# G1OJS/PyFT8

Hardware: AMD Instinct MI355X
Metric: FT8 15-s frames decoded/sec (higher is better)
Workload: dtype f32

## Files before the change

pyft8_amd/csrc/ft8rx.hip:

```cpp
#include <hip/hip_runtime.h>
#include <math.h>
#include <stdarg.h>
#include <stdio.h>
#include <stdlib.h>
#include <string.h>
#include <algorithm>
#include <map>
#include <new>
#include <string>
#include <vector>
#include "../../include/ft8rx.h"
#include "ft8_dev.h"

#define WL_MULT(i) ((i) == WL_BP0 ? 5 : (i) == WL_OSDNAN ? 10 : 1)
#define NF0MAX (FT8RX_MAX_F0 > 1024 ? 2048 : 1024)

#include "kernels/common.hpp"
#include "kernels/spectrogram.hpp"
#include "kernels/sync_search.hpp"
#include "kernels/llr.hpp"
#include "kernels/ap_patterns.hpp"
#include "kernels/bp.hpp"
#include "kernels/cycle_spectrum.hpp"
#include "kernels/fine_sync.hpp"
// ... 585 lines not shown
static void launch_ap_calls(ft8rx_handle* h, int B, const float* llr0, ft8rx_record* rec, const int32_t* ncand, Att* attO, ft8rx_event* ev,
                            int32_t* evc, int32_t* cand_items, int32_t* osd_items, int32_t* ac, const ApCalls* apc, hipStream_t s) {
    const ft8rx_config& c = h->cfg;
    const int sh = cand_shift(c); const size_t S = (size_t)1 << sh;
    const int nflip = osd_nflip(c.osd_single, c.osd_triple);
    hipMemsetAsync(ac, 0, 2 * sizeof(int32_t), s);
    const WorkList cl = {cand_items, ac}, ol = {osd_items, ac + 1};
    k_ap_worklist<<<(B * S + 255) / 256, 256, 0, s>>>(rec, ncand, B, sh, cl);
    k_bp_ap<<<ladder_grid(h, B * c.max_cands * h->ap.np), 64, 0, s>>>(llr0, rec, ncand, attO, ev, evc, c, apc, cl, ol);
    (osd_wide(nflip) ? k_osd_ap_wide : k_osd_ap)<<<ladder_grid(h, B * c.max_cands * 3), 64, 0, s>>>(
        llr0, rec, ncand, attO, ev, evc, h->d_trials, h->n_trials, nflip, sh, apc, ol);
    k_select_ap<<<(B * S + 255) / 256, 256, 0, s>>>(rec, attO, apc, cl);
}

static void launch_reports(ft8rx_handle* h, int B, const cpx* spec, const ft8rx_record* rec, const int32_t* ncand, int32_t* items,
                           int32_t* count, ft8rx_report* rep, hipStream_t s) {
    const ft8rx_config& c = h->cfg;
    const int sh = cand_shift(c); const size_t S = (size_t)1 << sh;
    hipMemsetAsync(count, 0, sizeof(int32_t), s);
    const WorkList wl = {items, count};
    k_report_worklist<<<(B * S + 255) / 256, 256, 0, s>>>(rec, ncand, B, sh, wl, rep);
    k_report<<<ladder_grid(h, B * c.max_cands), FINE_NT, 0, s>>>(spec, rec, rep, h->T, sh, wl);
}

static void enqueue_chain(ft8rx_handle* h, const int16_t* d_audio, int f0, int B, hipStream_t s, bool prof, int slot, int chunk) {
    const ResultSlot& sl = h->slots[slot];
    const bool weak = h->weak;
    const ft8rx_config cw = weak ? weak_config(h) : h->cfg;
    const ft8rx_config& c = weak ? cw : h->cfg;
    const size_t F = (size_t)f0;
    const int sh = cand_shift(c); const size_t S = (size_t)1 << sh, FS = F * S;
    const int16_t* audio = d_audio + F * FT8RX_NSAMP;
    float* grid = h->d_grid + F * FT8RX_GRID_ROWS * FT8RX_GRID_COLS;
    float* bs = h->d_best_score + F * NF0MAX; int32_t* bh = h->d_best_h0 + F * NF0MAX;
    ft8rx_record* rec = sl.rec + FS; int32_t* ncand = sl.ncand + F;
    float* llr0 = h->d_llr0 + FS * 174; float* saved = h->d_saved + FS * 5 * 174;
    Att* att0 = h->d_att0 + FS * 5; Att* attG = h->d_attG + FS * 2; Att* attB = h->d_attB + FS * 5; Att* attO = h->d_attO + FS * 10;
    cpx* A = reinterpret_cast<cpx*>(grid); cpx* spec = A + (size_t)B * 96000;
    ft8rx_event* ev = sl.ev + F * FT8RX_EVENT_CAP; int32_t* evc = sl.evcount + F;
#define STAGE(name) do { if (prof) { hipEventRecord(h->pev[h->pnames.size()], s); h->pnames.push_back(name); } } while (0)
    int32_t* wc = h->d_wcount + WL_N * chunk;
    WorkList wl[WL_N];
    for (int i = 0; i < WL_N; i++) { wl[i].items = h->d_work[i] + FS * WL_MULT(i); wl[i].count = wc + i; }
    STAGE("spectrogram");
    ft8rx_ilp_spectrogram(B, s, audio, grid, h->T);
    STAGE("sync");
    launch_sync(grid, bs, bh, c, B, s, weak);
    STAGE("topk");
    k_topk<<<B, 1024, 0, s>>>(bs, bh, rec, ncand, c, evc, wc, h->use_mask ? h->d_colmask + F * NF0MAX : nullptr);
    STAGE("grid_llr");
    const unsigned mt = (unsigned)h->msg_types;
    launch_mt(k_grid_llr, k_grid_llr_ext, mt, XCD_GRID(B, c.max_cands), s, grid, rec, ncand, llr0, c, nullptr, nullptr, nullptr, att0, ev, evc, B);
    k_worklist_att<<<(B * S * 5 + 255) / 256, 256, 0, s>>>(rec, ncand, att0, B, sh, wl[WL_BP0]);
    STAGE("bp_grid");
    launch_mt(k_bp, k_bp_ext, mt, ladder_grid(h, B * c.max_cands * 5), s, 0, llr0, rec, ncand, nullptr, att0, nullptr, ev, evc, c, c.bp_nc0_a, c.bp_iters_a, wl[WL_BP0], 0, 5);
    STAGE("select0");
    k_select0<<<(B * S + 255) / 256, 256, 0, s>>>(rec, ncand, att0, B, sh, wl[WL_FINE]);
    STAGE("cycle_fft");
    k_cyc_a<<<dim3(40, B), 256, 0, s>>>(audio, A, h->T);
    k_cyc_bc<<<dim3(CYC_BC_GRID, B), 256, 0, s>>>(A, spec, h->T);
    STAGE("fine");
    launch_fine(h, c, weak, ladder_grid(h, B * c.max_cands), s, spec, rec, ncand, llr0, nullptr, nullptr, nullptr, nullptr, wl[WL_FINE],
                c.h0_lo < FT8RX_MIN_H0_FD || c.h0_hi > FT8RX_MAX_H0_FD + 1);
    k_worklist<<<(B * S + 255) / 256, 256, 0, s>>>(rec, ncand, B, sh, wl[WL_BP1]);
    STAGE("bp_fine");
    const auto bp_fine = [&](int n_variants, const WorkList& work, int v0) {
        launch_mt(k_bp, k_bp_ext, mt, B * c.max_cands * n_variants, s, 1, llr0, rec, ncand, attG, attB, saved, ev, evc, c, c.bp_nc0_b, c.bp_iters_b,
                  work, v0, n_variants);
    };
    if (h->ladder_mode == 0) {
        bp_fine(1, wl[WL_BP1], 0);
        k_select1<<<(B * S + 255) / 256, 256, 0, s>>>(0, rec, ncand, attG, attB, B, c, wl[WL_BP1B]);
        bp_fine(1, wl[WL_BP1B], 1);
        k_select1<<<(B * S + 255) / 256, 256, 0, s>>>(1, rec, ncand, attG, attB, B, c, wl[WL_BP1C]);
        bp_fine(3, wl[WL_BP1C], 2);
        STAGE("select1");
        k_select1<<<(B * S + 255) / 256, 256, 0, s>>>(2, rec, ncand, attG, attB, B, c, wl[WL_OSD]);
    } else {
        bp_fine(5, wl[WL_BP1], 0);
        STAGE("select1");
        k_select1<<<(B * S + 255) / 256, 256, 0, s>>>(3, rec, ncand, attG, attB, B, c, wl[WL_OSD]);
    }
    STAGE("osd");
    launch_osd(h, mt, ladder_grid(h, B * c.max_cands * 10), s, 0, llr0, saved, attB, rec, ncand, attO, ev, evc, h->d_trials, h->n_trials,
               osd_nflip(c.osd_single, c.osd_triple), c.osd_max_hd, sh, wl[WL_OSD], wl[WL_OSDNAN]);
    STAGE("select2");
    k_select2<<<(B * S + 255) / 256, 256, 0, s>>>(rec, ncand, attO, B, sh);
    if (h->ap.np) {
        STAGE("ap_calls");
        ApCalls* apc = h->d_apc + chunk;
        if (h->ap_chunk_version[chunk] != h->ap_version) {
            k_ap_stage<<<1, 64, 0, s>>>(apc, h->ap);
            h->ap_chunk_version[chunk] = h->ap_version;
        }
        launch_ap_calls(h, B, llr0, rec, ncand, attO, ev, evc, wl[WL_BP0].items, wl[WL_OSDNAN].items, h->d_apcount + 2 * chunk, apc, s);
    }
    if (sl.recall) {
        STAGE("recall");
        ft8rx_recall_entry* ent = sl.d_rc_ent + F * FT8RX_RECALL_MAX;
        int32_t* rcnt = sl.d_rc_cnt + F;
        k_recall_stage<<<B, FT8RX_RECALL_MAX, 0, s>>>(h->d_rc_src + F * FT8RX_RECALL_MAX, h->d_rc_srccnt + F, ent, rcnt, sl.d_rc_rec + F * FT8RX_RECALL_MAX);
        const int base = h->rc_off[F], n = h->rc_off[F + B] - base;
        if (n > 0) {
            k_recall_trip<<<B, FT8RX_RECALL_MAX, 0, s>>>(ent, rcnt, h->d_rc_off + F, h->d_rc_trip);
            const size_t b = (size_t)base;
            launch_fine(h, c, false, n, s, spec, nullptr, nullptr, h->d_rc_llr + b * 174, h->d_rc_trip + 3 * b, h->d_rc_tout + 5 * b,
                        h->d_rc_tsd + b, h->d_rc_sgrid + b * 632, WorkList{nullptr, nullptr}, h->rc_td);
            k_recall_score<<<n, 64, 0, s>>>(h->d_rc_sgrid, h->d_rc_tout, h->d_rc_trip, h->d_rc_off + F, base, ent, rec, ncand, sh,
                                            h->rc_max_hd, h->rc_min_gap, sl.d_rc_rec + F * FT8RX_RECALL_MAX);
        }
    }
    if (sl.reports) {
        STAGE("report");
        launch_reports(h, B, spec, rec, ncand, h->d_rp_items + FS, h->d_rp_count + chunk, sl.d_rp + FS, s);
    }
    if (prof) hipEventRecord(h->pev[h->pnames.size()], s);
#undef STAGE
}

static void enqueue_chunk(ft8rx_handle* h, const int16_t* d_audio, int f0, int n, hipStream_t s, int slot, int chunk) {
    const int sub = (h->sub_frames > 0 && h->sub_frames < n) ? h->sub_frames : n;
    for (int o = 0; o < n; o += sub) enqueue_chain(h, d_audio, f0 + o, (o + sub <= n) ? sub : n - o, s, false, slot, chunk);
}

using batchplan::BatchPlan;
using batchplan::Entry;

static int batch_begin(ft8rx_handle* h, Entry e, int B, int slot, bool chunked, int16_t** stage) {
    ResultSlot& sl = h->slots[slot];
    h->pnames.clear();
    if (e != batchplan::DEVICE && need_staging(h)) return -2;
    if (e == batchplan::HOST_PIPELINED && slot == 1 && need_staging(h, true)) return -2;
    if (h->inflight == 2) { h->slot_fetch ^= 1; h->inflight = 1; }
    if (h->rc_armed && B != h->rc_frames) { set_err(h, "recall entries were set for %d frames, the batch has %d", h->rc_frames, B); return -1; }
    sl.recall = h->rc_armed;
    h->rc_armed = false;
    sl.reports = h->reports;
    *stage = h->d_audio;
    if (e == batchplan::HOST_PIPELINED) {
        *stage = slot ? h->d_audio2 : h->d_audio;
        HIPCHK(h, hipStreamWaitEvent(h->h2d_s, sl.ev_comp, 0));
    }
    for (int i = 1; i < h->n_streams && chunked; i++) if (!h->sub[i - 1]) {
        if (!(h->sub[i - 1] = pool_sub(h->device, i - 1))) { set_err(h, "cannot create a chunk stream"); return -2; }
        HIPCHK(h, hipEventCreateWithFlags(&h->ev_join[i - 1], hipEventDisableTiming));
    }
    return 0;
}

static int batch_submit(ft8rx_handle* h, const BatchPlan& plan, Entry e, int slot, const int16_t* audio, int16_t* stage) {
    ResultSlot& sl = h->slots[slot];
    const bool host = e != batchplan::DEVICE;
    const int16_t* d_audio = host ? stage : audio; const int16_t* host_audio = host ? audio : nullptr;
    const int ns = h->n_streams, nc = plan.nc, B = plan.cb[nc];
    const bool free_run = plan.mode == batchplan::FREE_RUN, pipelined = e == batchplan::HOST_PIPELINED, sync_host = e == batchplan::HOST_SYNC;
    hipStream_t cs = pipelined ? h->h2d_s : h->copy_s;
    const size_t frame_bytes = sizeof(int16_t) * (size_t)FT8RX_NSAMP;
    auto chunk_stream = [&](int k) { const int i = k % ns; return i == 0 ? h->stream : h->sub[i - 1]; };
    if (free_run) {
        for (int i = 0; i < ns; i++) for (int k = 0; k < 2; k++)
            if (!h->ev_cdone[k][i]) HIPCHK(h, hipEventCreateWithFlags(&h->ev_cdone[k][i], hipEventDisableTiming));
        if (h->need_barrier || h->part_B != B || h->part_n != nc) {
            if (h->free_running) HIPCHK(h, hipStreamWaitEvent(h->stream, h->slots[h->last_slot].ev_comp, 0));
            HIPCHK(h, hipEventRecord(h->ev_fork, h->stream));
            for (int i = 1; i < ns; i++) HIPCHK(h, hipStreamWaitEvent(h->sub[i - 1], h->ev_fork, 0));
            h->need_barrier = false; h->part_B = B; h->part_n = nc;
        }
// ... 2078 lines not shown
```

pyft8_amd/csrc/kernels/osd.hpp:

```cpp
#ifndef FT8RX_OSD_HPP
#define FT8RX_OSD_HPP

#ifdef OSD_TIMING
__device__ unsigned long long g_osd_t[32768][10];
struct OsdClock { unsigned long long prev = __builtin_readcyclecounter(); };
#define OT(i) do { const unsigned long long ot_now = __builtin_readcyclecounter(); if (lane == 0) g_osd_t[blockIdx.x & 32767][i] += ot_now - ot.prev; ot.prev = __builtin_readcyclecounter(); } while (0)
#define OT_FLUSH do { if (lane == 0) g_osd_t[blockIdx.x & 32767][9] += 1ull; } while (0)
#else
struct OsdClock {};
#define OT(i) do { } while (0)
#define OT_FLUSH do { } while (0)
#endif
template <int M> FT8_DEV uint32_t osd_px(uint32_t v, int lane) {
    if (M == 1) return (uint32_t)__builtin_amdgcn_update_dpp(0, (int)v, 0xB1, 0xf, 0xf, false);
    if (M == 2) return (uint32_t)__builtin_amdgcn_update_dpp(0, (int)v, 0x4E, 0xf, 0xf, false);
    if (M == 3) return (uint32_t)__builtin_amdgcn_update_dpp(0, (int)v, 0x1B, 0xf, 0xf, false);
    if (M == 7) return (uint32_t)__builtin_amdgcn_update_dpp(0, (int)v, 0x141, 0xf, 0xf, false);
    if (M == 15) return (uint32_t)__builtin_amdgcn_update_dpp(0, (int)v, 0x140, 0xf, 0xf, false);
    if (M == 8) return (uint32_t)__builtin_amdgcn_update_dpp(0, (int)v, 0x128, 0xf, 0xf, false);
    if (M == 4 || M == 16 || M == 31) return (uint32_t)__builtin_amdgcn_ds_swizzle((int)v, 0x1f | (M << 10));
    return __shfl(v, lane ^ M);
}
#define OSD_LOWMASK(top) ((top) == 1 ? 0x5555555555555555ull : (top) == 2 ? 0x3333333333333333ull : (top) == 4 ? 0x0F0F0F0F0F0F0F0Full : \
                          (top) == 8 ? 0x00FF00FF00FF00FFull : (top) == 16 ? 0x0000FFFF0000FFFFull : 0x00000000FFFFFFFFull)
// ... 47 lines not shown
    const int val = a[last]; int next = last - 1;
    while (osd_nl(x, val, a[next])) { a[last] = a[next]; last = next; next--; }
    a[last] = val;
}
FT8_HD void osd_ss_insertion(const float* x, int* a, int first, int last) {
    for (int i = first + 1; i < last; i++) {
        if (osd_nl(x, a[i], a[first])) { const int val = a[i]; for (int j = i; j > first; j--) a[j] = a[j - 1]; a[first] = val; }
        else osd_ss_linear_insert(x, a, i);
    }
}
FT8_HD void osd_ss_adjust_heap(const float* x, int* a, int first, int hole, int len, int value) {
    const int top = hole; int child = hole;
    while (child < (len - 1) / 2) {
        child = 2 * (child + 1);
        if (osd_nl(x, a[first + child], a[first + child - 1])) child--;
        a[first + hole] = a[first + child]; hole = child;
    }
    if ((len & 1) == 0 && child == (len - 2) / 2) { child = 2 * (child + 1); a[first + hole] = a[first + child - 1]; hole = child - 1; }
    int parent = (hole - 1) / 2;
    while (hole > top && osd_nl(x, a[first + parent], value)) { a[first + hole] = a[first + parent]; hole = parent; parent = (hole - 1) / 2; }
    a[first + hole] = value;
}
FT8_HD void osd_std_sort_withnan(const float* x, int* a, int* stack ) {
    const int n = 174;
    for (int i = 0; i < n; i++) a[i] = i;
    int sp = 0;
    stack[0] = 0; stack[1] = n; stack[2] = 2 * 7; sp = 1;
    while (sp > 0) {
        sp--;
        int first = stack[3 * sp], last = stack[3 * sp + 1], depth = stack[3 * sp + 2];
        while (last - first > 16) {
            if (depth == 0) {
                const int len = last - first;
                for (int parent = (len - 2) / 2; parent >= 0; parent--) osd_ss_adjust_heap(x, a, first, parent, len, a[first + parent]);
                while (last - first > 1) { last--; const int v = a[last]; a[last] = a[first]; osd_ss_adjust_heap(x, a, first, 0, last - first, v); }
                break;
            }
            depth--;
            {
                const int p = first + 1, q = first + (last - first) / 2, r = last - 1;
                int pick;
                if (osd_nl(x, a[p], a[q])) pick = osd_nl(x, a[q], a[r]) ? q : (osd_nl(x, a[p], a[r]) ? r : p);
                else pick = osd_nl(x, a[p], a[r]) ? p : (osd_nl(x, a[q], a[r]) ? r : q);
                const int t = a[first]; a[first] = a[pick]; a[pick] = t;
            }
            int lo = first + 1, hi = last;
            for (;;) {
                while (osd_nl(x, a[lo], a[first])) lo++;
                hi--;
                while (osd_nl(x, a[first], a[hi])) hi--;
                if (!(lo < hi)) break;
                const int t = a[lo]; a[lo] = a[hi]; a[hi] = t;
                lo++;
            }
            stack[3 * sp] = lo; stack[3 * sp + 1] = last; stack[3 * sp + 2] = depth; sp++;
            last = lo;
        }
    }
    osd_ss_insertion(x, a, 0, 16);
    for (int i = 16; i < n; i++) osd_ss_linear_insert(x, a, i);
}

#undef FT8_HD
__device__ uint8_t d_NANPERM[192];

#define OSD_MAXFLIP 91
#define OSD_FLIPS_A 62
#define OSD_MAXTRIALS 16384
#define OSD_NONE 0xFFu

__device__ __constant__ uint32_t d_SYNM[14][3];
__device__ uint32_t d_G0T[192][3];

struct OsdArgs {
    const float* llr_in; const float* saved; const Att* attB; ft8rx_record* rec; const int32_t* ncand; Att* attO;
    ft8rx_event* ev; int32_t* evcount; const uint32_t* trials; int ntr, nflip, max_hd, sh; WorkList nanlist; unsigned mt; const ApCalls* apc;
};

struct OsdLds {
    float llr[176];
    uint64_t work[256];
    uint64_t ftab[192];
    uint32_t hmw[3];
    uint16_t fsyn[OSD_MAXFLIP + 2];
    FT8_DEV int* ordl() { return reinterpret_cast<int*>(work); }
    FT8_DEV int* posrow() { return reinterpret_cast<int*>(work); }
    FT8_DEV uint32_t* ftabB() { return reinterpret_cast<uint32_t*>(work); }
    FT8_DEV int* frow() { return reinterpret_cast<int*>(work) + 192; }
};
static_assert(176 + 3 * 20 <= 512 && 192 + OSD_MAXFLIP <= 512 && sizeof(OsdLds) <= 4496, "the overlays fit the 512 words of work[]; 4.5 KB per block");

struct OsdInput { bool go; int slot; size_t vec; const float* hsrc; };
template <bool AP7>
FT8_DEV OsdInput osd_load(OsdLds& L, int lane, int mode, int bid, const OsdArgs& a) {
    OsdInput in = {true, 0, (size_t)bid, L.llr};
    if constexpr (AP7) {
        in.slot = bid & 15; const size_t c = (size_t)(bid >> 4);
        in.hsrc = a.llr_in + c * 174;
        const float v0 = in.hsrc[lane], v1 = in.hsrc[64 + lane], v2 = in.hsrc[128 + (lane < 46 ? lane : 0)];
        L.llr[lane] = ap7_value(a.apc, in.slot, lane, v0); L.llr[64 + lane] = ap7_value(a.apc, in.slot, 64 + lane, v1);
        if (lane < 46) L.llr[128 + lane] = ap7_value(a.apc, in.slot, 128 + lane, v2);
        in.vec = c * 10 + (in.slot - 5);
    } else if (mode == 0) {
        const int slot = in.slot = bid % 10; const int c = bid / 10;
        in.go = false;
        if ((c & ((1 << a.sh) - 1)) >= a.ncand[c >> a.sh]) return in;
        if (a.rec[c].status != FT8RX_ST_ACTIVE) return in;
        if (slot >= 5 && !a.attB[(size_t)c * 5 + (slot - 5)].has_out) { if (lane == 0) { Att u; memset(&u, 0, sizeof(u)); u.n_its = -1; a.attO[(size_t)c * 10 + slot] = u; } return in; }
        in.go = true;
        const float* src = slot < 5 ? a.llr_in + (size_t)c * 174 : a.saved + ((size_t)c * 5 + (slot - 5)) * 174;
        const int apx = slot < 5 ? slot : 0;
        const float v0 = src[lane], v1 = src[64 + lane], v2 = src[128 + (lane < 46 ? lane : 0)];
        L.llr[lane] = ap_value(apx, lane, v0); L.llr[64 + lane] = ap_value(apx, 64 + lane, v1);
        if (lane < 46) L.llr[128 + lane] = ap_value(apx, 128 + lane, v2);
        in.vec = (size_t)c * 10 + slot;
    } else {
        for (int i = lane; i < 174; i += 64) L.llr[i] = a.llr_in[in.vec * 174 + i];
    }
    __syncthreads();
    return in;
}

template <bool NANV>
FT8_DEV bool osd_order(OsdLds& L, int lane, int bid, const WorkList& nanlist, uint32_t* ix, OsdClock& ot) {
    uint32_t hk[3];
#pragma unroll
    for (int q = 0; q < 3; q++) {
        const int i = lane + 64 * q;
        const uint32_t mag = __float_as_uint(L.llr[i < 174 ? i : 0]) & 0x7fffffffu;
        hk[q] = (i < 174) ? 0xFFFFFFFEu - mag : 0xFFFFFFFFu;
        ix[q] = (i < 174) ? (uint32_t)i : 0u;
    }
    const uint64_t nan0 = __ballot(hk[0] < 0x807FFFFEu), nan1 = __ballot(hk[1] < 0x807FFFFEu), nan2 = __ballot(lane < 46 && hk[2] < 0x807FFFFEu);
    const bool any_nan = (nan0 | nan1 | nan2) != 0, all_nan = (nan0 & nan1) == ~0ull && nan2 == (1ull << 46) - 1;
    OT(0);
    if (NANV) {
        if (!any_nan || all_nan) return false;
        int* ordl = L.ordl();
        if (lane == 0) osd_std_sort_withnan(L.llr, ordl, ordl + 176);
        __syncthreads();
        ix[0] = (uint32_t)ordl[lane]; ix[1] = (uint32_t)ordl[64 + lane]; ix[2] = (uint32_t)ordl[128 + (lane < 46 ? lane : 0)];
        __syncthreads();
    } else if (all_nan) {
        ix[0] = d_NANPERM[lane]; ix[1] = d_NANPERM[64 + lane]; ix[2] = d_NANPERM[128 + lane];
    } else if (any_nan) {
        if (lane == 0) work_push(nanlist, bid);
        return false;
    } else {
        osd_stage<1, 3>(hk, ix, lane); osd_stage<3, 3>(hk, ix, lane); osd_stage<1, 3>(hk, ix, lane);
        osd_stage<7, 3>(hk, ix, lane); osd_stage<2, 3>(hk, ix, lane); osd_stage<1, 3>(hk, ix, lane);
        osd_stage<15, 3>(hk, ix, lane); osd_stages_421<3>(hk, ix, lane);
        osd_stage<31, 3>(hk, ix, lane); osd_stage<8, 3>(hk, ix, lane); osd_stages_421<3>(hk, ix, lane);
        osd_stage<63, 3>(hk, ix, lane); osd_stage<16, 3>(hk, ix, lane); osd_stage<8, 3>(hk, ix, lane); osd_stages_421<3>(hk, ix, lane);
        osd_stage_regs<true>(hk[0], ix[0], hk[1], ix[1], lane);
        osd_stage<32, 2>(hk, ix, lane); osd_stage<16, 2>(hk, ix, lane); osd_stage<8, 2>(hk, ix, lane); osd_stages_421<2>(hk, ix, lane);
        osd_stage_regs<true>(hk[1], ix[1], hk[2], ix[2], lane);
        osd_stage_regs<false>(hk[0], ix[0], hk[1], ix[1], lane);
        osd_stage<32, 3>(hk, ix, lane); osd_stage<16, 3>(hk, ix, lane); osd_stage<8, 3>(hk, ix, lane); osd_stages_421<3>(hk, ix, lane);
    }
    return true;
}

struct OsdHard { uint64_t w0, w1, w2; };
FT8_DEV OsdHard osd_hard(const float* v, int lane) {
    return {__ballot(v[lane] > 0.0f), __ballot(v[64 + lane] > 0.0f), __ballot(lane < 46 && v[128 + (lane < 46 ? lane : 0)] > 0.0f)};
}

struct OsdBasis {
    uint32_t x00, x01, x02, x10, x11, x12, x20, x21, x22;
    uint64_t acc0, acc1, acc2;
    bool hs0, hs1, hs2;
};
FT8_DEV OsdBasis osd_eliminate(OsdLds& L, int lane, const uint32_t* ix, OsdClock& ot) {
    const int ord0 = (int)ix[0], ord1 = (int)ix[1], ord2 = (lane < 46) ? (int)ix[2] : 0;
    const bool has2 = lane < 46;
    uint32_t x00 = d_G0T[ord0][0], x01 = d_G0T[ord0][1], x02 = d_G0T[ord0][2];
    uint32_t x10 = d_G0T[ord1][0], x11 = d_G0T[ord1][1], x12 = d_G0T[ord1][2];
    uint32_t x20 = has2 ? d_G0T[ord2][0] : 0u, x21 = has2 ? d_G0T[ord2][1] : 0u, x22 = has2 ? d_G0T[ord2][2] : 0u;
    const bool hs0 = L.llr[ord0] > 0.0f, hs1 = L.llr[ord1] > 0.0f, hs2 = has2 && L.llr[ord2] > 0.0f;
    uint64_t acc0 = 0, acc1 = 0, acc2 = 0;
    int k = 0;
#define OSD_TRIV 96
    int* posrow = L.posrow();
    if (ord0 < 91) posrow[ord0] = lane;
    if (ord1 < 91) posrow[ord1] = 64 + lane;
    if (has2 && ord2 < 91) posrow[ord2] = 128 + lane;
    uint64_t triv0 = __ballot(ord0 < 91), triv1 = __ballot(ord1 < 91 && lane < OSD_TRIV - 64);
    int tc0 = __builtin_amdgcn_mbcnt_hi((uint32_t)(triv0 >> 32), __builtin_amdgcn_mbcnt_lo((uint32_t)triv0, 0));
    int tc1 = __popcll(triv0) + __builtin_amdgcn_mbcnt_hi((uint32_t)(triv1 >> 32), __builtin_amdgcn_mbcnt_lo((uint32_t)triv1, 0));
    int ntriv = __popcll(triv0) + __popcll(triv1);
    __syncthreads();
    const uint64_t u01 = __ballot(posrow[lane] < OSD_TRIV);
    const uint32_t u2 = (uint32_t)__ballot(lane < 27 && posrow[64 + (lane < 27 ? lane : 0)] < OSD_TRIV);
    uint64_t vis0 = ~triv0, vis1 = ~triv1, vis2 = (1ull << 46) - 1;
#define OSD_UPD(XW, X0, X1, X2) { const uint32_t mk = (uint32_t)__builtin_amdgcn_sbfe((int)(XW), bp, 1u); X0 ^= mk & m0; X1 ^= mk & m1; X2 ^= mk & m2; }
#define OSD_STEP(XA, XB, XC, ACC, VIS, TCV, BASE, UPD0, UPD1, UPD2)                                                                \
    while (VIS != 0) {                                                                                                             \
        const int il = __builtin_ctzll(VIS);                                                                                       \
        if (k + __builtin_amdgcn_readlane(TCV, il) >= 91) { vis0 = 0; vis1 = 0; vis2 = 0; continue; }       \
        const uint64_t bit = 1ull << il;                                                                                           \
        VIS &= ~bit; ACC |= bit; k++;                                                                                              \
        const uint32_t c0 = __builtin_amdgcn_readlane(XA, il), c1 = __builtin_amdgcn_readlane(XB, il), c2 = __builtin_amdgcn_readlane(XC, il); \
        uint32_t a0 = c0 & ~lockU0, a1 = c1 & ~lockU1, a2 = c2 & ~lockU2;                                                          \
        if (__builtin_expect(!(a0 | a1 | a2), 0)) {             \
            const int p = (BASE) + il;                                                                                             \
             \
            const int pa = posrow[lane], pb = posrow[64 + (lane < 27 ? lane : 0)];                                                 \
            const bool ta = pa > p && pa < OSD_TRIV && (((pa < 64 ? triv0 >> pa : triv1 >> (pa - 64)) & 1ull) != 0);               \
            const bool tb = lane < 27 && pb > p && pb < OSD_TRIV && (((pb < 64 ? triv0 >> pb : triv1 >> (pb - 64)) & 1ull) != 0);  \
            const uint64_t s01 = (((uint64_t)c1 << 32) | c0) & __ballot(ta);                                                       \
            a0 = (uint32_t)s01; a1 = (uint32_t)(s01 >> 32); a2 = c2 & (uint32_t)__ballot(tb);                                      \
            if (a0 | a1 | a2) {                                                                                                    \
                const int r = s01 ? __builtin_ctzll(s01) : 64 + __builtin_ctz(a2);                                                 \
                const int q = __builtin_amdgcn_readfirstlane(posrow[r]);    \
                if (q < 64) { triv0 &= ~(1ull << q); vis0 |= 1ull << q; tc0 -= (lane > q) ? 1 : 0; tc1 -= 1; }                    \
                else { triv1 &= ~(1ull << (q - 64)); vis1 |= 1ull << (q - 64); tc1 -= (lane > q - 64) ? 1 : 0; }                   \
                ntriv--;                                                                                                           \
            } else { ACC &= ~bit; k--; }                                                    \
        }                                                                                                                          \
        asm volatile("" : "+s"(a2));                            \
                        \
        if (a0) {                                                                                                                  \
            const uint32_t b = a0 & (0u - a0), bp = __builtin_ctz(a0), m0 = c0 & ~b, m1 = c1, m2 = c2;                             \
            UPD0                                                                                                                   \
            lockU0 |= b;                                                                                                           \
        } else if (a1) {                                                                                                           \
            const uint32_t b = a1 & (0u - a1), bp = __builtin_ctz(a1), m0 = c0, m1 = c1 & ~b, m2 = c2;                             \
            UPD1                                                                                                                   \
            lockU1 |= b;                                                                                                           \
        } else {                                                \
            const uint32_t b = a2 & (0u - a2), bp = __builtin_ctz(a2 | 0x80000000u), m0 = c0, m1 = c1, m2 = c2 & ~b;               \
            UPD2                                                                                                                   \
            lockU2 |= b;                                                                                                           \
        }                                                                                                                          \
    }
    uint32_t lockU0 = (uint32_t)u01, lockU1 = (uint32_t)(u01 >> 32), lockU2 = ~((1u << 27) - 1u) | u2;
    OT(2);
    OSD_STEP(x00, x01, x02, acc0, vis0, tc0, 0,
             OSD_UPD(x00, x00, x01, x02) OSD_UPD(x10, x10, x11, x12) OSD_UPD(x20, x20, x21, x22),
             OSD_UPD(x01, x00, x01, x02) OSD_UPD(x11, x10, x11, x12) OSD_UPD(x21, x20, x21, x22),
             OSD_UPD(x02, x00, x01, x02) OSD_UPD(x12, x10, x11, x12) OSD_UPD(x22, x20, x21, x22))
    OSD_STEP(x10, x11, x12, acc1, vis1, tc1, 64,
             OSD_UPD(x10, x10, x11, x12) OSD_UPD(x20, x20, x21, x22),
             OSD_UPD(x11, x10, x11, x12) OSD_UPD(x21, x20, x21, x22),
             OSD_UPD(x12, x10, x11, x12) OSD_UPD(x22, x20, x21, x22))
    {
        int tc2 = ntriv;
        OSD_STEP(x20, x21, x22, acc2, vis2, tc2, 128, OSD_UPD(x20, x20, x21, x22), OSD_UPD(x21, x20, x21, x22), OSD_UPD(x22, x20, x21, x22))
    }
#undef OSD_STEP
#undef OSD_UPD
    acc0 |= __ballot(((triv0 >> lane) & 1ull) && tc0 < 91 - k);
    acc1 |= __ballot(((triv1 >> lane) & 1ull) && tc1 < 91 - k);
    __syncthreads();
    return {x00, x01, x02, x10, x11, x12, x20, x21, x22, acc0, acc1, acc2, hs0, hs1, hs2};
}

template <bool WIDE>
FT8_DEV void osd_flip_table(OsdLds& L, int lane, const uint32_t* ix, const OsdBasis& b, int nflip, OsdClock& ot) {
    const int nflipA = WIDE ? OSD_FLIPS_A : nflip;
    const bool has2 = lane < 46;
    const int ord0 = (int)ix[0], ord1 = (int)ix[1], ord2 = has2 ? (int)ix[2] : 0;
    const bool in0 = (b.acc0 >> lane) & 1ull, in1 = (b.acc1 >> lane) & 1ull, in2 = (b.acc2 >> lane) & 1ull;
    const int n0 = __popcll(b.acc0), n1 = __popcll(b.acc1);
    const int kk0 = __builtin_amdgcn_mbcnt_hi((uint32_t)(b.acc0 >> 32), __builtin_amdgcn_mbcnt_lo((uint32_t)b.acc0, 0));
    const int kk1 = n0 + __builtin_amdgcn_mbcnt_hi((uint32_t)(b.acc1 >> 32), __builtin_amdgcn_mbcnt_lo((uint32_t)b.acc1, 0));
    const int kk2 = n0 + n1 + __builtin_amdgcn_mbcnt_hi((uint32_t)(b.acc2 >> 32), __builtin_amdgcn_mbcnt_lo((uint32_t)b.acc2, 0));
    int* fri = L.frow();
#define OSD_ROWIDX(X0, X1, X2) ((X0) ? __builtin_ctz(X0) : (X1) ? 32 + __builtin_ctz(X1) : 64 + __builtin_ctz((X2) | 0x80000000u))
    { const int i = 90 - kk0; if (in0 && i >= 0 && i < nflip) fri[i] = OSD_ROWIDX(b.x00, b.x01, b.x02); }
    { const int i = 90 - kk1; if (in1 && i >= 0 && i < nflip) fri[i] = OSD_ROWIDX(b.x10, b.x11, b.x12); }
    { const int i = 90 - kk2; if (in2 && i >= 0 && i < nflip) fri[i] = OSD_ROWIDX(b.x20, b.x21, b.x22); }
#undef OSD_ROWIDX
    if (lane < 3) L.hmw[lane] = 0u;
    __syncthreads();
    {
        const uint32_t h0 = ((in0 && b.hs0) ? b.x00 : 0u) | ((in1 && b.hs1) ? b.x10 : 0u) | ((in2 && b.hs2) ? b.x20 : 0u);
        const uint32_t h1 = ((in0 && b.hs0) ? b.x01 : 0u) | ((in1 && b.hs1) ? b.x11 : 0u) | ((in2 && b.hs2) ? b.x21 : 0u);
        const uint32_t h2 = ((in0 && b.hs0) ? b.x02 : 0u) | ((in1 && b.hs1) ? b.x12 : 0u) | ((in2 && b.hs2) ? b.x22 : 0u);
        if (h0) atomicOr(&L.hmw[0], h0);
        if (h1) atomicOr(&L.hmw[1], h1);
        if (h2) atomicOr(&L.hmw[2], h2);
    }
    __syncthreads();
    const uint32_t hm0 = L.hmw[0], hm1 = L.hmw[1], hm2 = L.hmw[2];
    OT(4);
    uint32_t f0l = 0, f1l = 0, f2l = 0;
    uint32_t f0h = (uint32_t)((__popc(b.x00 & hm0) + __popc(b.x01 & hm1) + __popc(b.x02 & hm2)) & 1) << 31,
             f1h = (uint32_t)((__popc(b.x10 & hm0) + __popc(b.x11 & hm1) + __popc(b.x12 & hm2)) & 1) << 31,
             f2h = (uint32_t)((__popc(b.x20 & hm0) + __popc(b.x21 & hm1) + __popc(b.x22 & hm2)) & 1) << 31;
#define OSD_FBIT(XA, XB, XC, FA, FB, FC, SH) { FA |= __builtin_amdgcn_ubfe(XA, bp, 1u) << (SH); FB |= __builtin_amdgcn_ubfe(XB, bp, 1u) << (SH); \
                                               FC |= __builtin_amdgcn_ubfe(XC, bp, 1u) << (SH); }
#define OSD_FLIPS(LO, HI, FA, FB, FC, SUB)                                                                                         \
    for (int i = (LO); i < (HI); i++) {                                                                                            \
        const int r = __builtin_amdgcn_readfirstlane(fri[i]);                                                                      \
        const uint32_t bp = (uint32_t)r & 31u, sh = (uint32_t)(i - (SUB));                                                         \
        if (r < 32) OSD_FBIT(b.x00, b.x10, b.x20, FA, FB, FC, sh)                                                                  \
        else if (r < 64) OSD_FBIT(b.x01, b.x11, b.x21, FA, FB, FC, sh)                                                             \
        else OSD_FBIT(b.x02, b.x12, b.x22, FA, FB, FC, sh)                                                                         \
    }
    OSD_FLIPS(0, nflipA < 32 ? nflipA : 32, f0l, f1l, f2l, 0)
    OSD_FLIPS(32, nflipA, f0h, f1h, f2h, 32)
    L.ftab[ord0] = ((uint64_t)f0h << 32) | f0l; L.ftab[ord1] = ((uint64_t)f1h << 32) | f1l; if (has2) L.ftab[ord2] = ((uint64_t)f2h << 32) | f2l;
    if (WIDE) {
        uint32_t* ftabB = L.ftabB();
        uint32_t g0 = 0, g1 = 0, g2 = 0;
        OSD_FLIPS(OSD_FLIPS_A, nflip, g0, g1, g2, OSD_FLIPS_A)
        ftabB[ord0] = g0; ftabB[ord1] = g1; if (has2) ftabB[ord2] = g2;
    }
#undef OSD_FLIPS
#undef OSD_FBIT
    __syncthreads();
}

template <class Bit> FT8_DEV unsigned osd_syndrome_of(Bit bit) {
    uint32_t ra = 0, rb = 0, rc = 0;
#pragma unroll 8
    for (int v = 0; v < 32; v++) { ra |= bit(v) << v; rb |= bit(32 + v) << v; rc |= bit(64 + (v < 27 ? v : 0)) << v; }
    rc &= (1u << 27) - 1;
    unsigned sy = 0;
#pragma unroll
    for (int k = 0; k < 14; k++)
        sy |= (unsigned)((__popc(ra & d_SYNM[k][0]) + __popc(rb & d_SYNM[k][1]) + __popc(rc & d_SYNM[k][2])) & 1) << k;
    return sy;
}
template <bool WIDE>
FT8_DEV void osd_syndromes(OsdLds& L, int lane, int nflip) {
    const int nflipA = WIDE ? OSD_FLIPS_A : nflip;
    const int bitsel = (lane < nflipA) ? lane : 63;
    const uint32_t* fh = reinterpret_cast<const uint32_t*>(L.ftab) + (bitsel >= 32 ? 1 : 0);
    const unsigned sy = osd_syndrome_of([&](int v) { return __builtin_amdgcn_ubfe(fh[2 * v], (uint32_t)bitsel & 31u, 1u); });
    if (lane < nflipA) L.fsyn[lane] = (uint16_t)sy;
    if (lane == 63) L.fsyn[OSD_MAXFLIP + 1] = (uint16_t)sy;
    if (lane == 0) L.fsyn[OSD_MAXFLIP] = 0;
    if (WIDE) {
        const uint32_t* ftabB = L.ftabB();
        const unsigned syB = osd_syndrome_of([&](int v) { return (ftabB[v] >> (lane & 31)) & 1u; });
        if (OSD_FLIPS_A + lane < nflip) L.fsyn[OSD_FLIPS_A + lane] = (uint16_t)syB;
    }
    __syncthreads();
}

template <bool WIDE, bool EXT, bool AP7>
FT8_DEV Att osd_trials(OsdLds& L, int lane, const OsdInput& in, const OsdHard& hard, const OsdArgs& a) {
    const bool has2 = lane < 46;
    const uint32_t* ftabB = L.ftabB();
    const unsigned syn_c = L.fsyn[OSD_MAXFLIP + 1];
    const uint64_t M1 = (1ull << 27) - 1, M2 = (1ull << 46) - 1;
    Att res; memset(&res, 0, sizeof(res)); res.n_its = -1;
    const int slot = in.slot, ipass = AP7 ? 7 : (slot < 5) ? 5 : 6;
    for (int base = 0; base < a.ntr; base += 64) {
        const int t = base + lane;
        bool hit = false; int i = OSD_MAXFLIP, j = OSD_MAXFLIP, q = OSD_MAXFLIP;
        if (t < a.ntr) {
            const uint32_t e = a.trials[t];
            i = e & 0xFF; j = (e >> 8) & 0xFF; q = (e >> 16) & 0xFF;
            if (i == OSD_NONE) i = OSD_MAXFLIP;
            if (j == OSD_NONE) j = OSD_MAXFLIP;
            if (q == OSD_NONE) q = OSD_MAXFLIP;
            hit = (syn_c ^ L.fsyn[i] ^ L.fsyn[j] ^ L.fsyn[q]) == 0;
        }
        uint64_t hits = __ballot(hit);
        if (!hits) continue;
        bool done = false;
        while (hits && !done) {
            const int hl = __builtin_ctzll(hits);
            hits &= hits - 1;
            const int hi_ = __shfl(i, hl), hj = __shfl(j, hl), hq = __shfl(q, hl);
            const uint64_t msk = (1ull << 63) | ((hi_ < OSD_FLIPS_A) ? (1ull << hi_) : 0ull) | ((hj < OSD_FLIPS_A) ? (1ull << hj) : 0ull) |
                                 ((hq < OSD_FLIPS_A) ? (1ull << hq) : 0ull);
            uint32_t mskB = 0;
            if (WIDE) mskB = ((hi_ >= OSD_FLIPS_A && hi_ < OSD_MAXFLIP) ? (1u << (hi_ - OSD_FLIPS_A)) : 0u) |
                             ((hj >= OSD_FLIPS_A && hj < OSD_MAXFLIP) ? (1u << (hj - OSD_FLIPS_A)) : 0u) |
                             ((hq >= OSD_FLIPS_A && hq < OSD_MAXFLIP) ? (1u << (hq - OSD_FLIPS_A)) : 0u);
            const int l2 = 128 + (has2 ? lane : 0);
            const int pb0 = WIDE ? __popc(ftabB[lane] & mskB) : 0, pb1 = WIDE ? __popc(ftabB[64 + lane] & mskB) : 0, pb2 = WIDE ? __popc(ftabB[l2] & mskB) : 0;
            const uint64_t w0 = __ballot((__popcll(L.ftab[lane] & msk) + pb0) & 1), w1 = __ballot((__popcll(L.ftab[64 + lane] & msk) + pb1) & 1),
                           w2 = __ballot(has2 && ((__popcll(L.ftab[l2] & msk) + pb2) & 1));
            const int hd = __popcll(w0 ^ hard.w0) + __popcll(w1 ^ hard.w1) + __popcll((w2 ^ hard.w2) & M2);
            if (a.max_hd > 0 && hd > a.max_hd) continue;
            uint64_t lo = 0, hi = 0;
            const int r = ft8_crc_check<EXT>(w0, w1 & M1, &lo, &hi, a.mt, true);
            const int t = base + hl;
            if (r && lane == 0) log_event(a.ev, a.evcount, (int)(in.vec / 10) >> a.sh, (int)(in.vec / 10) & ((1 << a.sh) - 1), ipass, AP7 ? 2 * slot + 1 : slot, t, lo, hi, r == 2);
            if (r == 2) {
                res.ok = 1; res.lo = lo; res.hi = hi; res.n_its = (int16_t)t;
                if constexpr (AP7) res.ok = hd <= a.apc->max_hd;
                res.method = (AP7 || slot < 5) ? FT8RX_M_OSD : FT8RX_M_LDPC_B_OSD;
                res.pad[0] = (uint8_t)hd;
                done = true;
            }
        }
        if (done) break;
    }
    return res;
}

template <bool WIDE, bool NANV, bool EXT = false, bool AP7 = false>
FT8_DEV void osd_attempt(int lane, int mode, int bid, const OsdArgs& a) {
    __shared__ OsdLds L;
    OsdClock ot;
    const OsdInput in = osd_load<AP7>(L, lane, mode, bid, a);
    if (!in.go) return;
    uint32_t ix[3];
    if (!osd_order<NANV>(L, lane, bid, a.nanlist, ix, ot)) return;
    OT(1);
    const OsdHard hard = osd_hard(in.hsrc, lane);
    const OsdBasis basis = osd_eliminate(L, lane, ix, ot);
    OT(3);
    osd_flip_table<WIDE>(L, lane, ix, basis, a.nflip, ot);
    OT(5);
    osd_syndromes<WIDE>(L, lane, a.nflip);
    OT(6);
    const Att res = osd_trials<WIDE, EXT, AP7>(L, lane, in, hard, a);
    OT(7);
    if (lane == 0) a.attO[in.vec] = res;
    OT_FLUSH;
}

#ifndef OSD_ATTR
#define OSD_ATTR __attribute__((amdgpu_waves_per_eu(8, 8)))
#endif
template <bool WIDE, bool NANV, bool EXT, bool AP7, class Id>
FT8_DEV void osd_blocks(int n, int mode, const OsdArgs& a, Id id) {
#pragma unroll 1
    for (int item = blockIdx.x; item < n; item += gridDim.x) {
        int lane = threadIdx.x;
        asm volatile("" : "+v"(lane));
        osd_attempt<WIDE, NANV, EXT, AP7>(lane, mode, id(item), a);
        __syncthreads();
    }
}
#define OSD_PARAMS int mode, const float* __restrict__ llr_in, const float* __restrict__ saved, const Att* __restrict__ attB,       \
                   ft8rx_record* __restrict__ rec, const int32_t* __restrict__ ncand, Att* __restrict__ attO, ft8rx_event* ev,      \
                   int32_t* evcount, const uint32_t* __restrict__ trials, int ntr, int nflip, int max_hd, int sh
#define OSD_KERNEL(NAME, NAN_NAME, WIDE, EXT, MT_PARAM, MT)                                                                          \
__global__ __launch_bounds__(64) OSD_ATTR void NAME(OSD_PARAMS, WorkList work, WorkList nanlist MT_PARAM) {                         \
    const OsdArgs a = {llr_in, saved, attB, rec, ncand, attO, ev, evcount, trials, ntr, nflip, max_hd, sh, nanlist, MT, nullptr};   \
    osd_blocks<WIDE, false, EXT, false>(mode == 2 ? (int)gridDim.x : *work.count * 10, mode, a,                                     \
                                        [&](int item) { return mode == 2 ? item : work.items[item / 10] * 10 + item % 10; });       \
}                                                                                                                                   \
__global__ __launch_bounds__(64) void NAN_NAME(OSD_PARAMS, WorkList nanlist MT_PARAM) {                                             \
    const OsdArgs a = {llr_in, saved, attB, rec, ncand, attO, ev, evcount, trials, ntr, nflip, max_hd, sh, nanlist, MT, nullptr};   \
    osd_blocks<WIDE, true, EXT, false>(*nanlist.count, mode, a, [&](int item) { return nanlist.items[item]; });                     \
}
#define OSD_MT_PARAM , unsigned mt
OSD_KERNEL(k_osd, k_osd_nan, false, false, , 0u)
OSD_KERNEL(k_osd_wide, k_osd_nan_wide, true, false, , 0u)
OSD_KERNEL(k_osd_ext, k_osd_nan_ext, false, true, OSD_MT_PARAM, mt)
OSD_KERNEL(k_osd_wide_ext, k_osd_nan_wide_ext, true, true, OSD_MT_PARAM, mt)
#undef OSD_KERNEL
#undef OSD_PARAMS
#undef OSD_MT_PARAM
#define OSD_NAN_GRID 512

#endif
```

Before: 88820.

## Fuse OSD AP slots 2-4 into one block sharing Gaussian elimination

The OSD kernel now handles AP slots 2, 3 and 4 of a candidate in a single block. The ordering, elimination, flip table and syndromes are computed once for slot 2. Slots 3 and 4 are expressed as codeword deltas, built from the AP_END pattern bits and stored in spare ftabB bits, and the trial search is then rerun per pass with adjusted hard bits and masks. This cuts OSD work items from 10 to 8 per candidate and removes the repeated elimination, at the cost of more LDS atomics, extra trial passes inside one block, and a correctness risk if the delta encoding is wrong.

```diff
diff --git a/pyft8_amd/csrc/ft8rx.hip b/pyft8_amd/csrc/ft8rx.hip
--- a/pyft8_amd/csrc/ft8rx.hip
+++ b/pyft8_amd/csrc/ft8rx.hip
@@ -691,7 +691,7 @@
         k_select1<<<(B * S + 255) / 256, 256, 0, s>>>(3, rec, ncand, attG, attB, B, c, wl[WL_OSD]);
     }
     STAGE("osd");
-    launch_osd(h, mt, ladder_grid(h, B * c.max_cands * 10), s, 0, llr0, saved, attB, rec, ncand, attO, ev, evc, h->d_trials, h->n_trials,
+    launch_osd(h, mt, ladder_grid(h, B * c.max_cands * OSD_ITEMS), s, 0, llr0, saved, attB, rec, ncand, attO, ev, evc, h->d_trials, h->n_trials,
                osd_nflip(c.osd_single, c.osd_triple), c.osd_max_hd, sh, wl[WL_OSD], wl[WL_OSDNAN]);
     STAGE("select2");
     k_select2<<<(B * S + 255) / 256, 256, 0, s>>>(rec, ncand, attO, B, sh);
diff --git a/pyft8_amd/csrc/kernels/osd.hpp b/pyft8_amd/csrc/kernels/osd.hpp
--- a/pyft8_amd/csrc/kernels/osd.hpp
+++ b/pyft8_amd/csrc/kernels/osd.hpp
@@ -153,13 +153,15 @@
     uint64_t work[256];
     uint64_t ftab[192];
     uint32_t hmw[3];
-    uint16_t fsyn[OSD_MAXFLIP + 2];
+    uint16_t fsyn[OSD_MAXFLIP + 4];
     FT8_DEV int* ordl() { return reinterpret_cast<int*>(work); }
     FT8_DEV int* posrow() { return reinterpret_cast<int*>(work); }
     FT8_DEV uint32_t* ftabB() { return reinterpret_cast<uint32_t*>(work); }
     FT8_DEV int* frow() { return reinterpret_cast<int*>(work) + 192; }
+    FT8_DEV uint32_t* hmd() { return reinterpret_cast<uint32_t*>(work) + 288; }
 };
-static_assert(176 + 3 * 20 <= 512 && 192 + OSD_MAXFLIP <= 512 && sizeof(OsdLds) <= 4496, "the overlays fit the 512 words of work[]; 4.5 KB per block");
+static_assert(176 + 3 * 20 <= 512 && 192 + OSD_MAXFLIP <= 288 && 288 + 8 <= 512 && sizeof(OsdLds) <= 4496, "the overlays fit the 512 words of work[]; 4.5 KB per block");
+#define OSD_CWB 29
 
 struct OsdInput { bool go; int slot; size_t vec; const float* hsrc; };
 template <bool AP7>
@@ -193,7 +195,7 @@
 }
 
 template <bool NANV>
-FT8_DEV bool osd_order(OsdLds& L, int lane, int bid, const WorkList& nanlist, uint32_t* ix, OsdClock& ot) {
+FT8_DEV bool osd_order(OsdLds& L, int lane, int bid, int nids, const WorkList& nanlist, uint32_t* ix, OsdClock& ot) {
     uint32_t hk[3];
 #pragma unroll
     for (int q = 0; q < 3; q++) {
@@ -215,7 +217,7 @@
     } else if (all_nan) {
         ix[0] = d_NANPERM[lane]; ix[1] = d_NANPERM[64 + lane]; ix[2] = d_NANPERM[128 + lane];
     } else if (any_nan) {
-        if (lane == 0) work_push(nanlist, bid);
+        if (lane == 0) for (int k = 0; k < nids; k++) work_push(nanlist, bid + k);
         return false;
     } else {
         osd_stage<1, 3>(hk, ix, lane); osd_stage<3, 3>(hk, ix, lane); osd_stage<1, 3>(hk, ix, lane);
@@ -327,8 +329,15 @@
     return {x00, x01, x02, x10, x11, x12, x20, x21, x22, acc0, acc1, acc2, hs0, hs1, hs2};
 }
 
+struct OsdTriple { bool on; uint32_t d3, d4; };
+FT8_DEV OsdTriple osd_triple(int lane) {
+    const uint64_t p = __ballot(lane < 57 && (&d_AP_END[0][0])[lane < 57 ? lane : 0] != 0);
+    const uint32_t p2 = (uint32_t)p & 0x7FFFFu, p3 = (uint32_t)(p >> 19) & 0x7FFFFu, p4 = (uint32_t)(p >> 38);
+    return {true, p2 ^ p3, p2 ^ p4};
+}
+
 template <bool WIDE>
-FT8_DEV void osd_flip_table(OsdLds& L, int lane, const uint32_t* ix, const OsdBasis& b, int nflip, OsdClock& ot) {
+FT8_DEV void osd_flip_table(OsdLds& L, int lane, const uint32_t* ix, const OsdBasis& b, int nflip, bool triple, OsdClock& ot) {
     const int nflipA = WIDE ? OSD_FLIPS_A : nflip;
     const bool has2 = lane < 46;
     const int ord0 = (int)ix[0], ord1 = (int)ix[1], ord2 = has2 ? (int)ix[2] : 0;
@@ -343,7 +352,10 @@
     { const int i = 90 - kk1; if (in1 && i >= 0 && i < nflip) fri[i] = OSD_ROWIDX(b.x10, b.x11, b.x12); }
     { const int i = 90 - kk2; if (in2 && i >= 0 && i < nflip) fri[i] = OSD_ROWIDX(b.x20, b.x21, b.x22); }
 #undef OSD_ROWIDX
+    uint32_t* hmd = L.hmd();
+    const OsdTriple tri = triple ? osd_triple(lane) : OsdTriple{false, 0u, 0u};
     if (lane < 3) L.hmw[lane] = 0u;
+    if (tri.on && lane < 8) hmd[lane] = lane < 6 ? 0u : lane == 6 ? tri.d3 : tri.d3 ^ tri.d4;
     __syncthreads();
     {
         const uint32_t h0 = ((in0 && b.hs0) ? b.x00 : 0u) | ((in1 && b.hs1) ? b.x10 : 0u) | ((in2 && b.hs2) ? b.x20 : 0u);
@@ -353,6 +365,20 @@
         if (h1) atomicOr(&L.hmw[1], h1);
         if (h2) atomicOr(&L.hmw[2], h2);
     }
+    if (tri.on) {
+        const uint32_t i0 = (uint32_t)ord0 - 58u, i1 = (uint32_t)ord1 - 58u, i2 = (uint32_t)ord2 - 58u;
+        const bool a0 = in0 && i0 < 19u, a1 = in1 && i1 < 19u, a2 = in2 && i2 < 19u;
+#pragma unroll
+        for (int s = 0; s < 2; s++) {
+            const uint32_t d = s ? tri.d4 : tri.d3;
+            const bool t0 = a0 && ((d >> (i0 & 31u)) & 1u), t1 = a1 && ((d >> (i1 & 31u)) & 1u), t2 = a2 && ((d >> (i2 & 31u)) & 1u);
+            if (t0 || t1 || t2) {
+                atomicOr(&hmd[3 * s + 0], (t0 ? b.x00 : 0u) | (t1 ? b.x10 : 0u) | (t2 ? b.x20 : 0u));
+                atomicOr(&hmd[3 * s + 1], (t0 ? b.x01 : 0u) | (t1 ? b.x11 : 0u) | (t2 ? b.x21 : 0u));
+                atomicOr(&hmd[3 * s + 2], (t0 ? b.x02 : 0u) | (t1 ? b.x12 : 0u) | (t2 ? b.x22 : 0u));
+            }
+        }
+    }
     __syncthreads();
     const uint32_t hm0 = L.hmw[0], hm1 = L.hmw[1], hm2 = L.hmw[2];
     OT(4);
@@ -360,6 +386,14 @@
     uint32_t f0h = (uint32_t)((__popc(b.x00 & hm0) + __popc(b.x01 & hm1) + __popc(b.x02 & hm2)) & 1) << 31,
              f1h = (uint32_t)((__popc(b.x10 & hm0) + __popc(b.x11 & hm1) + __popc(b.x12 & hm2)) & 1) << 31,
              f2h = (uint32_t)((__popc(b.x20 & hm0) + __popc(b.x21 & hm1) + __popc(b.x22 & hm2)) & 1) << 31;
+    uint32_t* ftabB = L.ftabB();
+    if (tri.on) {
+        const uint32_t k0 = hm0 ^ hmd[0], k1 = hm1 ^ hmd[1], k2 = hm2 ^ hmd[2], m0 = hm0 ^ hmd[3], m1 = hm1 ^ hmd[4], m2 = hm2 ^ hmd[5];
+#define OSD_CW2(XA, XB, XC) ((uint32_t)((__popc((XA) & k0) + __popc((XB) & k1) + __popc((XC) & k2)) & 1) << OSD_CWB | \
+                             (uint32_t)((__popc((XA) & m0) + __popc((XB) & m1) + __popc((XC) & m2)) & 1) << (OSD_CWB + 1))
+        ftabB[ord0] = OSD_CW2(b.x00, b.x01, b.x02); ftabB[ord1] = OSD_CW2(b.x10, b.x11, b.x12); if (has2) ftabB[ord2] = OSD_CW2(b.x20, b.x21, b.x22);
+#undef OSD_CW2
+    }
 #define OSD_FBIT(XA, XB, XC, FA, FB, FC, SH) { FA |= __builtin_amdgcn_ubfe(XA, bp, 1u) << (SH); FB |= __builtin_amdgcn_ubfe(XB, bp, 1u) << (SH); \
                                                FC |= __builtin_amdgcn_ubfe(XC, bp, 1u) << (SH); }
 #define OSD_FLIPS(LO, HI, FA, FB, FC, SUB)                                                                                         \
@@ -370,14 +404,16 @@
         else if (r < 64) OSD_FBIT(b.x01, b.x11, b.x21, FA, FB, FC, sh)                                                             \
         else OSD_FBIT(b.x02, b.x12, b.x22, FA, FB, FC, sh)                                                                         \
     }
+    uint32_t* fth = reinterpret_cast<uint32_t*>(L.ftab);
     OSD_FLIPS(0, nflipA < 32 ? nflipA : 32, f0l, f1l, f2l, 0)
+    fth[2 * ord0] = f0l; fth[2 * ord1] = f1l; if (has2) fth[2 * ord2] = f2l;
     OSD_FLIPS(32, nflipA, f0h, f1h, f2h, 32)
-    L.ftab[ord0] = ((uint64_t)f0h << 32) | f0l; L.ftab[ord1] = ((uint64_t)f1h << 32) | f1l; if (has2) L.ftab[ord2] = ((uint64_t)f2h << 32) | f2l;
+    fth[2 * ord0 + 1] = f0h; fth[2 * ord1 + 1] = f1h; if (has2) fth[2 * ord2 + 1] = f2h;
     if (WIDE) {
-        uint32_t* ftabB = L.ftabB();
         uint32_t g0 = 0, g1 = 0, g2 = 0;
         OSD_FLIPS(OSD_FLIPS_A, nflip, g0, g1, g2, OSD_FLIPS_A)
-        ftabB[ord0] = g0; ftabB[ord1] = g1; if (has2) ftabB[ord2] = g2;
+        if (tri.on) { atomicOr(&ftabB[ord0], g0); atomicOr(&ftabB[ord1], g1); if (has2) atomicOr(&ftabB[ord2], g2); }
+        else { ftabB[ord0] = g0; ftabB[ord1] = g1; if (has2) ftabB[ord2] = g2; }
     }
 #undef OSD_FLIPS
 #undef OSD_FBIT
@@ -396,7 +432,7 @@
     return sy;
 }
 template <bool WIDE>
-FT8_DEV void osd_syndromes(OsdLds& L, int lane, int nflip) {
+FT8_DEV void osd_syndromes(OsdLds& L, int lane, int nflip, bool triple) {
     const int nflipA = WIDE ? OSD_FLIPS_A : nflip;
     const int bitsel = (lane < nflipA) ? lane : 63;
     const uint32_t* fh = reinterpret_cast<const uint32_t*>(L.ftab) + (bitsel >= 32 ? 1 : 0);
@@ -404,19 +440,20 @@
     if (lane < nflipA) L.fsyn[lane] = (uint16_t)sy;
     if (lane == 63) L.fsyn[OSD_MAXFLIP + 1] = (uint16_t)sy;
     if (lane == 0) L.fsyn[OSD_MAXFLIP] = 0;
-    if (WIDE) {
+    if (WIDE || triple) {
         const uint32_t* ftabB = L.ftabB();
         const unsigned syB = osd_syndrome_of([&](int v) { return (ftabB[v] >> (lane & 31)) & 1u; });
-        if (OSD_FLIPS_A + lane < nflip) L.fsyn[OSD_FLIPS_A + lane] = (uint16_t)syB;
+        if (WIDE && OSD_FLIPS_A + lane < nflip) L.fsyn[OSD_FLIPS_A + lane] = (uint16_t)syB;
+        if (triple && (lane == OSD_CWB || lane == OSD_CWB + 1)) L.fsyn[OSD_MAXFLIP + 2 + (lane - OSD_CWB)] = (uint16_t)syB;
     }
     __syncthreads();
 }
 
 template <bool WIDE, bool EXT, bool AP7>
-FT8_DEV Att osd_trials(OsdLds& L, int lane, const OsdInput& in, const OsdHard& hard, const OsdArgs& a) {
+FT8_DEV Att osd_trials(OsdLds& L, int lane, const OsdInput& in, const OsdHard& hard, const OsdArgs& a, int pass) {
     const bool has2 = lane < 46;
     const uint32_t* ftabB = L.ftabB();
-    const unsigned syn_c = L.fsyn[OSD_MAXFLIP + 1];
+    const unsigned syn_c = L.fsyn[OSD_MAXFLIP + 1 + pass];
     const uint64_t M1 = (1ull << 27) - 1, M2 = (1ull << 46) - 1;
     Att res; memset(&res, 0, sizeof(res)); res.n_its = -1;
     const int slot = in.slot, ipass = AP7 ? 7 : (slot < 5) ? 5 : 6;
@@ -438,14 +475,15 @@
             const int hl = __builtin_ctzll(hits);
             hits &= hits - 1;
             const int hi_ = __shfl(i, hl), hj = __shfl(j, hl), hq = __shfl(q, hl);
-            const uint64_t msk = (1ull << 63) | ((hi_ < OSD_FLIPS_A) ? (1ull << hi_) : 0ull) | ((hj < OSD_FLIPS_A) ? (1ull << hj) : 0ull) |
+            const uint64_t msk = (pass ? 0ull : 1ull << 63) | ((hi_ < OSD_FLIPS_A) ? (1ull << hi_) : 0ull) | ((hj < OSD_FLIPS_A) ? (1ull << hj) : 0ull) |
                                  ((hq < OSD_FLIPS_A) ? (1ull << hq) : 0ull);
-            uint32_t mskB = 0;
-            if (WIDE) mskB = ((hi_ >= OSD_FLIPS_A && hi_ < OSD_MAXFLIP) ? (1u << (hi_ - OSD_FLIPS_A)) : 0u) |
-                             ((hj >= OSD_FLIPS_A && hj < OSD_MAXFLIP) ? (1u << (hj - OSD_FLIPS_A)) : 0u) |
-                             ((hq >= OSD_FLIPS_A && hq < OSD_MAXFLIP) ? (1u << (hq - OSD_FLIPS_A)) : 0u);
+            uint32_t mskB = pass ? 1u << (OSD_CWB - 1 + pass) : 0u;
+            if (WIDE) mskB |= ((hi_ >= OSD_FLIPS_A && hi_ < OSD_MAXFLIP) ? (1u << (hi_ - OSD_FLIPS_A)) : 0u) |
+                              ((hj >= OSD_FLIPS_A && hj < OSD_MAXFLIP) ? (1u << (hj - OSD_FLIPS_A)) : 0u) |
+                              ((hq >= OSD_FLIPS_A && hq < OSD_MAXFLIP) ? (1u << (hq - OSD_FLIPS_A)) : 0u);
             const int l2 = 128 + (has2 ? lane : 0);
-            const int pb0 = WIDE ? __popc(ftabB[lane] & mskB) : 0, pb1 = WIDE ? __popc(ftabB[64 + lane] & mskB) : 0, pb2 = WIDE ? __popc(ftabB[l2] & mskB) : 0;
+            const bool useB = WIDE || pass;
+            const int pb0 = useB ? __popc(ftabB[lane] & mskB) : 0, pb1 = useB ? __popc(ftabB[64 + lane] & mskB) : 0, pb2 = useB ? __popc(ftabB[l2] & mskB) : 0;
             const uint64_t w0 = __ballot((__popcll(L.ftab[lane] & msk) + pb0) & 1), w1 = __ballot((__popcll(L.ftab[64 + lane] & msk) + pb1) & 1),
                            w2 = __ballot(has2 && ((__popcll(L.ftab[l2] & msk) + pb2) & 1));
             const int hd = __popcll(w0 ^ hard.w0) + __popcll(w1 ^ hard.w1) + __popcll((w2 ^ hard.w2) & M2);
@@ -473,19 +511,26 @@
     OsdClock ot;
     const OsdInput in = osd_load<AP7>(L, lane, mode, bid, a);
     if (!in.go) return;
+    const bool triple = !NANV && !AP7 && mode == 0 && in.slot == 2;
     uint32_t ix[3];
-    if (!osd_order<NANV>(L, lane, bid, a.nanlist, ix, ot)) return;
+    if (!osd_order<NANV>(L, lane, bid, triple ? 3 : 1, a.nanlist, ix, ot)) return;
     OT(1);
-    const OsdHard hard = osd_hard(in.hsrc, lane);
+    OsdHard hard = osd_hard(in.hsrc, lane);
     const OsdBasis basis = osd_eliminate(L, lane, ix, ot);
     OT(3);
-    osd_flip_table<WIDE>(L, lane, ix, basis, a.nflip, ot);
+    osd_flip_table<WIDE>(L, lane, ix, basis, a.nflip, triple, ot);
     OT(5);
-    osd_syndromes<WIDE>(L, lane, a.nflip);
+    osd_syndromes<WIDE>(L, lane, a.nflip, triple);
     OT(6);
-    const Att res = osd_trials<WIDE, EXT, AP7>(L, lane, in, hard, a);
+    OsdInput ip = in;
+#pragma unroll 1
+    for (int pass = 0; pass < (triple ? 3 : 1); pass++, ip.slot++, ip.vec++) {
+        const uint32_t d = pass ? (uint32_t)__builtin_amdgcn_readfirstlane((int)L.hmd()[5 + pass]) : 0u;
+        hard.w0 ^= (uint64_t)(d & 63u) << 58; hard.w1 ^= (uint64_t)(d >> 6);
+        const Att res = osd_trials<WIDE, EXT, AP7>(L, lane, ip, hard, a, pass);
+        if (lane == 0) a.attO[ip.vec] = res;
+    }
     OT(7);
-    if (lane == 0) a.attO[in.vec] = res;
     OT_FLUSH;
 }
 
@@ -508,14 +553,17 @@
 #define OSD_KERNEL(NAME, NAN_NAME, WIDE, EXT, MT_PARAM, MT)                                                                          \
 __global__ __launch_bounds__(64) OSD_ATTR void NAME(OSD_PARAMS, WorkList work, WorkList nanlist MT_PARAM) {                         \
     const OsdArgs a = {llr_in, saved, attB, rec, ncand, attO, ev, evcount, trials, ntr, nflip, max_hd, sh, nanlist, MT, nullptr};   \
-    osd_blocks<WIDE, false, EXT, false>(mode == 2 ? (int)gridDim.x : *work.count * 10, mode, a,                                     \
-                                        [&](int item) { return mode == 2 ? item : work.items[item / 10] * 10 + item % 10; });       \
+    osd_blocks<WIDE, false, EXT, false>(mode == 2 ? (int)gridDim.x : *work.count * OSD_ITEMS, mode, a, [&](int item) {              \
+        if (mode == 2) return item;                                                                                                 \
+        const int q = item / OSD_ITEMS, j = (item + (int)((uint32_t)q * 0x9E3779B1u >> 29)) % OSD_ITEMS;            \
+        return work.items[q] * 10 + (j < 3 ? j : j + 2); });                                                                        \
 }                                                                                                                                   \
 __global__ __launch_bounds__(64) void NAN_NAME(OSD_PARAMS, WorkList nanlist MT_PARAM) {                                             \
     const OsdArgs a = {llr_in, saved, attB, rec, ncand, attO, ev, evcount, trials, ntr, nflip, max_hd, sh, nanlist, MT, nullptr};   \
     osd_blocks<WIDE, true, EXT, false>(*nanlist.count, mode, a, [&](int item) { return nanlist.items[item]; });                     \
 }
 #define OSD_MT_PARAM , unsigned mt
+#define OSD_ITEMS 8
 OSD_KERNEL(k_osd, k_osd_nan, false, false, , 0u)
 OSD_KERNEL(k_osd_wide, k_osd_nan_wide, true, false, , 0u)
 OSD_KERNEL(k_osd_ext, k_osd_nan_ext, false, true, OSD_MT_PARAM, mt)
```

Result: faster. 91170 (median of 6 runs) (+2.6%).
